# ielab/llm-rankers

Hardware: AMD Instinct MI355X
Metric: passages/sec (pointwise yes_no reranking, flan-t5-large shape) (higher is better)
Workload: dtype f16 (MFMA inputs), f32 accumulate + residual stream

## Files before the change

llm-rankers_amd/csrc/gemm.h:

```cpp
#pragma once
#include "common.h"
#include <type_traits>

enum GemmEpi { EPI_STORE_F16 = 0, EPI_RESID_F32 = 1, EPI_GEGLU_F16 = 2, EPI_RELU_F16 = 3, EPI_STORE_F32 = 4, EPI_SWIGLU_F16 = 5,
               EPI_ARGMAX_F32 = 6,
               EPI_LSE_F32 = 7 };
#define EPI_IS_GATED(E) ((E) == EPI_GEGLU_F16 || (E) == EPI_SWIGLU_F16)

struct GemmArgs {
  const half_t* A;
  const half_t* W;
  void* C;
  int lda, ldw, ldc;
  int M, N, K;
  int n_split;
  long split_stride;
  float scale;
  long bsA, bsW, bsC;
  const float* rowscale;
  half_t* xraw; float* ssq; int ldx, nb; float xs;
  const float* ssq_in; int nb_in; float eps_in;
  int* amax_idx;
  const int* lse_labels; int lse_npos; float* lse_xlab;
  int group_n;
// ... 371 lines not shown
      }
#pragma unroll
      for (int ni = 0; ni < 2; ++ni)
#pragma unroll
        for (int mi = 0; mi < 2; ++mi)
          acc[ni][mi] = __builtin_amdgcn_mfma_f32_32x32x16_f16(wf[ni], af[mi], acc[ni][mi], 0, 0, 0);
    }
    if (!GLDS && more) {
      gemm_write_tile(nA, wave, lane, ra);
      gemm_write_tile(nW, wave, lane, rw);
    }
  }

  if (EPI == EPI_RESID_F32) {
#pragma unroll
    for (int i = 0; i < 2; ++i)
#pragma unroll
      for (int j = 0; j < 2; ++j)
#pragma unroll
        for (int r = 0; r < 16; ++r) acc[i][j][r] = acc[i][j][r] * p.scale + res[i][j][r];
  }
  __syncthreads();
  if (EPI == EPI_RESID_F32) {
    GemmArgs q = p; q.scale = 1.f;
    float rsc[2] = {1.f, 1.f};
    gemm_epilogue_staged<EPI, 2, 2, true>(q, acc, m0 + wm * 64, n0 + wn * 64, lane, gemm_smem + wave * (32 * (64 * 4 + 16)), rsc);
  } else {
    float rsc[2];
    gemm_row_factors<2>(p, m0 + wm * 64, l31, rsc);
    gemm_epilogue_staged<EPI, 2, 2>(p, acc, m0 + wm * 64, n0 + wn * 64, lane, gemm_smem + wave * (32 * (64 * 4 + 16)), rsc);
  }
}

template <int EPI, int NST>
__global__ __launch_bounds__(128, NST == 4 ? 2 : (NST == 3 ? 3 : 4)) void gemm_s64_kernel(GemmArgs p) {
  extern __shared__ __attribute__((aligned(16))) unsigned char gemm_smem[];
  half_t* smem = (half_t*)gemm_smem;
  constexpr int TILE = 64 * 64;
  const int tid = threadIdx.x, lane = tid & 63;
  const int wave = __builtin_amdgcn_readfirstlane(tid >> 6);
  const int l31 = lane & 31, hh = lane >> 5;
  const int tiles_m = (p.M + 63) >> 6, tiles_n = (p.N + 63) >> 6;
  int tm, tn;
  gemm_tile_coords(blockIdx.x, tiles_m, tiles_n, tm, tn);
  const int m0 = tm * 64, n0 = tn * 64;
  const half_t* srcA[4];
  const half_t* srcW[4];
#pragma unroll
  for (int i = 0; i < 4; ++i) {
    const int pslot = (wave * 4 + i) * 64 + lane;
    const int r = pslot >> 3, c = pslot & 7;
    const int sw = (c ^ ((r >> 1) & 7)) << 3;
    const int ga = m0 + r < p.M ? m0 + r : p.M - 1, gw = n0 + r < p.N ? n0 + r : p.N - 1;
    srcA[i] = p.A + (size_t)ga * p.lda + sw;
    srcW[i] = p.W + (size_t)gw * p.ldw + sw;
  }
  auto stage = [&](int buf, int kt) {
    half_t* sA = smem + buf * 2 * TILE;
#pragma unroll
    for (int i = 0; i < 4; ++i)
      __builtin_amdgcn_global_load_lds((const __attribute__((address_space(1))) void*)(srcA[i] + kt * 64),
                                       (__attribute__((address_space(3))) void*)(sA + (wave * 4 + i) * 512), 16, 0, 0);
#pragma unroll
    for (int i = 0; i < 4; ++i)
      __builtin_amdgcn_global_load_lds((const __attribute__((address_space(1))) void*)(srcW[i] + kt * 64),
                                       (__attribute__((address_space(3))) void*)(sA + TILE + (wave * 4 + i) * 512), 16, 0, 0);
  };
  f32x16 acc[2][1];
#pragma unroll
  for (int i = 0; i < 2; ++i)
#pragma unroll
    for (int r = 0; r < 16; ++r) acc[i][0][r] = 0.f;
  const int nk = p.K >> 6;
#pragma unroll
  for (int s = 0; s < NST - 1; ++s)
    if (s < nk) stage(s, s);
  int cur = 0, nxt = NST - 1;
  for (int kt = 0; kt < nk; ++kt) {
    const int younger = nk - 1 - kt < NST - 2 ? nk - 1 - kt : NST - 2;
    if (younger >= 2) asm volatile("s_waitcnt vmcnt(16)" ::: "memory");
    else if (younger == 1) asm volatile("s_waitcnt vmcnt(8)" ::: "memory");
    else asm volatile("s_waitcnt vmcnt(0)" ::: "memory");
    __builtin_amdgcn_s_barrier();
    __builtin_amdgcn_sched_barrier(0);
    if (kt + NST - 1 < nk) stage(nxt, kt + NST - 1);
    const half_t* sA = smem + cur * 2 * TILE;
    const half_t* sW = sA + TILE;
#pragma unroll
    for (int ks = 0; ks < 4; ++ks) {
      const int cc = ks * 2 + hh;
      const half8 af = gemm_frag(sA, wave * 32 + l31, cc);
#pragma unroll
      for (int ni = 0; ni < 2; ++ni)
        acc[ni][0] = __builtin_amdgcn_mfma_f32_32x32x16_f16(gemm_frag(sW, ni * 32 + l31, cc), af, acc[ni][0], 0, 0, 0);
    }
    cur = cur + 1 == NST ? 0 : cur + 1;
    nxt = nxt + 1 == NST ? 0 : nxt + 1;
  }
  __syncthreads();
  float rsc[1];
  gemm_row_factors<1>(p, m0 + wave * 32, l31, rsc);
  gemm_epilogue_staged<EPI, 2, 1>(p, acc, m0 + wave * 32, n0, lane, gemm_smem + wave * (32 * (64 * 4 + 16)), rsc);
}

#define SKINNY_THREADS 512
template <int EPI, int NT>
__global__ __launch_bounds__(SKINNY_THREADS) void gemm_skinny_kernel(GemmArgs p) {
  __shared__ float red[4 * NT * 1024];
  const int tid = threadIdx.x, wave = tid >> 6, lane = tid & 63;
  const int l31 = lane & 31, hh = lane >> 5;
  const int n0 = blockIdx.x * 32 * NT;
  const int nsteps = p.K >> 4;
  const int mrow0 = blockIdx.z * 32;
  const int m = mrow0 + l31 < p.M ? mrow0 + l31 : p.M - 1;
  p.A += (size_t)blockIdx.y * p.bsA;
  p.W += (size_t)blockIdx.y * p.bsW;
  p.C = (char*)p.C + (size_t)blockIdx.y * p.bsC * ((EPI == EPI_RESID_F32 || EPI == EPI_STORE_F32 || EPI == EPI_ARGMAX_F32) ? 4 : 2);
  const half_t* arow = p.A + (size_t)m * p.lda + 8 * hh;
  const half_t* wrow[NT];
#pragma unroll
  for (int t = 0; t < NT; ++t) {
    int n = n0 + t * 32 + l31;
    n = n < p.N ? n : p.N - 1;
    wrow[t] = p.W + (size_t)n * p.ldw + 8 * hh;
  }
  f32x16 acc[NT][1];
#pragma unroll
  for (int t = 0; t < NT; ++t)
#pragma unroll
    for (int r = 0; r < 16; ++r) acc[t][0][r] = 0.f;
// ... 548 lines not shown
```

llm-rankers_amd/csrc/rk_engine.hip:

```cpp
#include <hip/hip_runtime.h>
#include <dlfcn.h>
#include <rccl/rccl.h>

#include <algorithm>
#include <cmath>
#include <cstdarg>
#include <cstdio>
#include <cstring>
#include <map>
#include <atomic>
#include <string>
#include <vector>

#include "../../include/rk_engine.h"
#include "attention.h"
#include "decoder_kernels.h"
#include "gemm.h"
#include "gemv_rows.h"
#include "llama_kernels.h"
#include "misc_kernels.h"

namespace {

thread_local std::string g_create_error;
// ... 43 lines not shown
  float* dhidden = nullptr; half_t *dxn = nullptr, *dqkv = nullptr, *dctx = nullptr, *dq = nullptr, *dffh = nullptr, *dlast = nullptr;
  half_t* dxraw[2] = {nullptr, nullptr}; float* dssq[2] = {nullptr, nullptr}; float* drowscale = nullptr;
  float* dssq_few[2] = {nullptr, nullptr};
  half_t *xqk = nullptr, *xctx = nullptr;
  float *xpart = nullptr, *xstat = nullptr; bool have_cross_kv = false;
  float* d_scores = nullptr; float* h_scores = nullptr;
  int* h_small = nullptr;
  std::vector<int> cache_dec, cache_out, cache_rows;
  std::vector<int> cache_g2; unsigned long dec_epoch = 0, g2_epoch = ~0ul;
  hipEvent_t ev_enc = nullptr, ev_dec = nullptr; bool dec_pending = false;
};

struct rk_engine {
  rk_model_desc d{};
  int dev = 0;
  std::string err;
  bool finalized = false;
  int inner = 0;
  std::map<std::string, HostTensor> host;
  std::vector<void*> allocs;
  half_t *emb = nullptr, *lm_head = nullptr, *cross_kv_w = nullptr;
  std::vector<EncLayerW> enc;
  std::vector<DecLayerW> dec;
  float *enc_final_ln = nullptr, *dec_final_ln = nullptr, *lut_enc = nullptr, *lut_dec = nullptr;
  float* logits = nullptr; size_t logits_cap = 0;
  const int* lse_labels = nullptr; int lse_npos = 0; float* lse_xlab = nullptr;
  float* amax_val = nullptr; int* amax_idx = nullptr; size_t amax_rows = 0;
  size_t scores_cap = 0;
  Slot slots[RK_SLOTS];
  struct Options {
    int glds = 1, skinny = 0x3F, overlap = 1, gemm_variant = 0, attn_short = 5, xattn_direct = 1, attn_heads_per_wg = 0, attn_ko = 0,
        gemm_persistent = 1, fold_norm = 1, s64_stages = 0, dec_fold_norm = 1, greedy_spec = 160, consumer_stats = 1, xattn_mfma = 1,
        dec_ffn_tiled = 1, gemm_split = 1, dec_fuse = 1, dec_fuse_rows = 0, dec_attn_seq = 1, attn_long = 1, attn_long_nw = 0,
        llama_attn_dma = 1, attn_long_xcd = 1, llama_attn_nw = 0, dec_graph = 1, gemm_sk = 1, dec_cross_mfma = 1, dec_gemv = 1, dec_gemv_rows = 4;
  } opt;
  float* attn_trace = nullptr;
  int n_cu = 256;
  struct SkWs { hipStream_t st = nullptr; float* slabs = nullptr; int* cnt = nullptr; };
  SkWs sk_ws[2 * RK_SLOTS];
  hipEvent_t t0 = nullptr, t1 = nullptr, t_tmp = nullptr;
  bool prof_on = false;
  std::vector<ProfRec> prof_recs; size_t prof_used = 0;
  double prof_flops[PC_COUNT] = {0}, prof_bytes[PC_COUNT] = {0}; int64_t prof_n[PC_COUNT] = {0};
  int family = 0; rk_llama_desc ld{};
  float rope_factor = 0.f, rope_low = 1.f, rope_high = 4.f; int rope_orig = 0;
  std::vector<LlamaLayerW> ll; float *l_final_ln = nullptr, *rope_cos = nullptr, *rope_sin = nullptr; int* d_pos = nullptr;
  struct GraphEntry { int seen = 0; bool failed = false; hipGraphExec_t exec = nullptr; };
  std::map<std::vector<int>, GraphEntry> graphs; int opt_epoch = 0;
  ncclComm_t comm = nullptr; int comm_rank = 0, comm_world = 1;
  float* d_gather[RK_SLOTS] = {nullptr}; float* h_gather[RK_SLOTS] = {nullptr}; size_t gather_cap = 0;
  hipEvent_t ev_gather[RK_SLOTS] = {nullptr}; bool gather_pending[RK_SLOTS] = {false}; int gather_n[RK_SLOTS] = {0};
  float *d_gsend = nullptr, *d_gall = nullptr, *h_gall = nullptr, *h_gstage = nullptr;
  hipEvent_t ev_gall = nullptr, ev_append = nullptr; bool gall_pending = false, append_foreign = false; int gall_n = 0;
};

namespace {

int fail(rk_engine* e, int code, const char* fmt, ...) {
  char buf[1024];
  va_list ap;
  va_start(ap, fmt);
  vsnprintf(buf, sizeof buf, fmt, ap);
  va_end(ap);
  if (e) e->err = buf; else g_create_error = buf;
  return code;
}

// ... 54 lines not shown
template <int EPI, int WM, int WN, int MI, int NI>
void launch_v2(hipStream_t st, const GemmArgs& a) {
  constexpr int BM = WM * MI * 32, BN = WN * NI * 32;
  constexpr int smem_stages = 2 * (BM + BN) * 64 * 2, smem_epi = WM * WN * 32 * (NI * 32 * 4 + 16);
  constexpr int smem = smem_stages > smem_epi ? smem_stages : smem_epi;
  static std::atomic<uint64_t> attr_done{0};
  ensure_dynamic_lds((const void*)gemm_v2_kernel<EPI, WM, WN, MI, NI>, smem, attr_done);
  const int tiles = ((a.M + BM - 1) / BM) * ((a.N + BN - 1) / BN);
  hipLaunchKernelGGL((gemm_v2_kernel<EPI, WM, WN, MI, NI>), dim3(tiles), dim3(WM * WN * 64), smem, st, a);
}

#define KSPLIT_MAX_SLABS 256

template <int EPI, int KO = 0, bool RS = false, bool SPLIT = false>
void launch_pp2(hipStream_t st, const GemmArgs& a, int max_wgs) {
  constexpr int smem = 2 * 4 * 128 * 64 * 2 + 32768;
  static std::atomic<uint64_t> attr_done{0};
  ensure_dynamic_lds((const void*)gemm_pp2_kernel<EPI, KO, RS, SPLIT>, smem, attr_done);
  const int tiles = ((a.M + 255) / 256) * ((a.N + 255) / 256) * (SPLIT ? a.ksplit : 1);
  const int grid = max_wgs > 0 && tiles > max_wgs ? max_wgs : tiles;
  hipLaunchKernelGGL((gemm_pp2_kernel<EPI, KO, RS, SPLIT>), dim3(grid), dim3(512), smem, st, a);
}

int choose_ksplit(const rk_engine* e, int epi, int M, int N, int K) {
  if (!e->opt.gemm_sk || !(epi == EPI_RESID_F32 || epi == EPI_STORE_F32) || K % 64) return 1;
  const long tiles = (long)((M + 255) / 256) * ((N + 255) / 256);
  const int wgs = e->n_cu & ~7, nk = K / 64;
  if (e->opt.gemm_sk == 2)
    return (nk >= 4 && tiles * 2 <= KSPLIT_MAX_SLABS) ? 2 : 1;
  if (epi != EPI_RESID_F32 || tiles < 1 || tiles * 2 > wgs || nk < 96) return 1;
  return 2;
}

int choose_variant(const rk_engine* e, int epi, int M, int N, int K, bool fold_producer, double* cost_out) {
  *cost_out = 0;
  if (e->opt.gemm_variant) return (e->opt.gemm_variant == 3 && (EPI_IS_GATED(epi) || fold_producer)) ? 2 : e->opt.gemm_variant;
  struct V { int id, bm, bn, slots; double round_us; };
  static const V vs[5] = {{5, 256, 256, 256, 25.5}, {2, 256, 256, 256, 29.8}, {3, 256, 192, 256, 24.7}, {4, 256, 128, 256, 19.0}, {1, 128, 128, 512, 17.3}};
  if ((long)((M + 127) / 128) * ((N + 127) / 128) <= 192 && K >= 64) { *cost_out = 15.0; return 6; }
  double best = 1e30; int bv = 1;
  for (const V& v : vs) {
    if (v.id == 3 && (EPI_IS_GATED(epi) || fold_producer)) continue;
    if (v.id == 5 && K < 128) continue;
    const long tiles = (long)((M + v.bm - 1) / v.bm) * ((N + v.bn - 1) / v.bn);
    double cost = (double)((tiles + v.slots - 1) / v.slots) * v.round_us;
    if (v.id == 5 && e->opt.gemm_sk == 1 && choose_ksplit(e, epi, M, N, K) > 1) cost = 0.0;
    if (cost < best - 1e-9) { best = cost; bv = v.id; }
  }
  *cost_out = best;
  return bv;
}

#define RK_XRAW_SCALE 0.0625f
struct GemmFold { const float* rowscale = nullptr; half_t* xraw = nullptr; float* ssq = nullptr; const float* ssq_in = nullptr; int nb_in = 0; };

enum GemmFamily { GEMM_NONE = -1, GEMM_TILED, GEMM_STREAM, GEMM_GEMV };
constexpr bool gemv_has(int E) { return E == EPI_STORE_F16 || E == EPI_RESID_F32 || E == EPI_GEGLU_F16 || E == EPI_RELU_F16 || E == EPI_STORE_F32; }
constexpr bool stream_has(int E) { return E != EPI_LSE_F32; }
constexpr bool tiled_has(int E) { return E != EPI_ARGMAX_F32; }
inline bool gemv_fits(int M, int K) { return M <= GEMV_MAX_ROWS && K % 8 == 0 && K <= 512 * GEMV_MAX_PIECES; }

struct Gemm {
  int cls, epi; const half_t* A; int lda; const half_t* W; int ldw; void* C; int ldc, M, N, K;
  int n_split = 0; long split_stride = 0;
  int batch = 1; long bsA = 0, bsW = 0, bsC = 0;
  GemmFamily family = GEMM_TILED;
  GemmFold fold;
  Gemm(int cls_, int epi_, const half_t* A_, int lda_, const half_t* W_, int ldw_, void* C_, int ldc_, int M_, int N_, int K_)
      : cls(cls_), epi(epi_), A(A_), lda(lda_), W(W_), ldw(ldw_), C(C_), ldc(ldc_), M(M_), N(N_), K(K_) {}
  Gemm& heads(int b, long sA, long sW, long sC) { batch = b; bsA = sA; bsW = sW; bsC = sC; return *this; }
  Gemm& split(int n, long stride) { n_split = n; split_stride = stride; return *this; }
  Gemm& on(GemmFamily f) { family = f; return *this; }
  Gemm& with(const GemmFold& f) { fold = f; return *this; }
};

struct GemmPlan {
  GemmFamily family = GEMM_NONE;
  int nb = 0;
  int m_pp2 = 0, ks_pp2 = 1, variant = 0, ksplit = 1, stages = 0;
  int wgs = 0;
  int ko = 0;
  const rk_engine::SkWs* ks_ws = nullptr;
  bool pp2() const { return family == GEMM_TILED && (m_pp2 > 0 || variant == 5); }
};

GemmPlan plan_gemm(const rk_engine* e, const Gemm& c, hipStream_t st) {
  GemmPlan p;
  const int epi = c.epi, M = c.M, N = c.N, K = c.K;
  if (c.family == GEMM_GEMV) {
    if (gemv_has(epi) && gemv_fits(M, K) && c.batch == 1 && c.n_split == 0) {
      p.family = GEMM_GEMV;
      p.nb = gemv_grid(N, e->n_cu);
    }
    return p;
  }
  if ((c.family == GEMM_STREAM || c.batch > 1) && c.n_split == 0 && (((e->opt.skinny >> epi) & 1) || c.batch > 1 || epi == EPI_ARGMAX_F32)) {
    if (stream_has(epi)) { p.family = GEMM_STREAM; p.nb = (N + 31) / 32; }
    return p;
  }
  if (!tiled_has(epi)) return p;
  p.family = GEMM_TILED;
  p.nb = (N + 63) / 64;
  p.wgs = e->opt.gemm_persistent == 1 ? (e->n_cu & ~7) : (e->opt.gemm_persistent & ~7);
  for (const auto& w : e->sk_ws) if (!p.ks_ws && w.st == st && w.slabs) p.ks_ws = &w;
  auto ksplit = [&](int rows) { return e->opt.gemm_persistent == 1 && p.ks_ws ? choose_ksplit(e, epi, rows, N, K) : 1; };
  const bool fold_producer = c.fold.xraw != nullptr;
  double whole = 0;
  p.variant = choose_variant(e, epi, M, N, K, fold_producer, &whole);
  if (e->opt.gemm_split && !e->opt.gemm_variant && K >= 128 && e->opt.gemm_persistent == 1 &&
      (epi == EPI_STORE_F16 || epi == EPI_RESID_F32 || EPI_IS_GATED(epi) || epi == EPI_RELU_F16)) {
    const int tiles_n = (N + 255) / 256, tiles_m = (M + 255) / 256;
    const long rounds = (long)tiles_m * tiles_n / p.wgs;
    const int panels = (int)(rounds * p.wgs / tiles_n);
    if (rounds >= 1 && (long)tiles_m * tiles_n % p.wgs != 0 && panels >= 1 && panels < tiles_m) {
      const long used = (long)panels * tiles_n;
      double rest = 0;
      const int v_rest = choose_variant(e, epi, M - panels * 256, N, K, fold_producer, &rest);
      if ((double)((used + p.wgs - 1) / p.wgs) * 25.5 + rest + 1.5 < whole - 1e-9) {
        p.m_pp2 = panels * 256; p.ks_pp2 = ksplit(p.m_pp2); p.variant = v_rest;
      }
    }
  }
#ifdef RK_MEASURE
  if (epi == EPI_STORE_F16 && p.variant > 80 && p.variant <= 96 && K >= 128) { p.ko = p.variant - 80; p.variant = 5; return p; }
#endif
  if (p.variant > 6) p.variant = 5;
  if (p.variant == 5 && K < 128) p.variant = 2;
  if (p.variant == 5) p.ksplit = ksplit(M - p.m_pp2);
  if (p.variant == 6) {
    const int tiles = ((M - p.m_pp2 + 63) / 64) * ((N + 63) / 64);
    p.stages = e->opt.s64_stages;
    if (p.stages < 2 || p.stages > 4) p.stages = tiles <= 2 * e->n_cu ? 4 : (tiles <= 3 * e->n_cu ? 3 : 2);
  }
  return p;
}

template <int EPI, int NST>
void launch_s64(hipStream_t st, const GemmArgs& a) {
  constexpr int smem = NST * 16384;
  static std::atomic<uint64_t> attr_done{0};
  ensure_dynamic_lds((const void*)gemm_s64_kernel<EPI, NST>, smem, attr_done);
  hipLaunchKernelGGL((gemm_s64_kernel<EPI, NST>), dim3(((a.M + 63) / 64) * ((a.N + 63) / 64)), dim3(128), smem, st, a);
}

template <int EPI>
void launch_pp2_plan(hipStream_t st, GemmArgs a, const GemmPlan& p, int ks) {
#ifdef RK_MEASURE
  if constexpr (EPI == EPI_STORE_F16) {
    switch (p.ko) {
      case 0: break;
      case 8: launch_pp2<EPI, 8>(st, a, p.wgs); return;
      case 16: launch_pp2<EPI, 16>(st, a, p.wgs); return;
      case 1: launch_pp2<EPI, 1>(st, a, p.wgs); return;
      case 2: launch_pp2<EPI, 2>(st, a, p.wgs); return;
      case 3: launch_pp2<EPI, 3>(st, a, p.wgs); return;
      case 4: launch_pp2<EPI, 4>(st, a, p.wgs); return;
      case 5: launch_pp2<EPI, 5>(st, a, p.wgs); return;
      default: launch_pp2<EPI, 6>(st, a, p.wgs); return;
    }
  }
#endif
  if constexpr (EPI == EPI_STORE_F16 || EPI_IS_GATED(EPI) || EPI == EPI_RELU_F16) {
    if (a.rowscale) { launch_pp2<EPI, 0, true>(st, a, p.wgs); return; }
  }
  if constexpr (EPI == EPI_RESID_F32 || EPI == EPI_STORE_F32) {
    if (ks > 1) { a.ksplit = ks; a.ks_slabs = p.ks_ws->slabs; a.ks_cnt = p.ks_ws->cnt; launch_pp2<EPI, 0, false, true>(st, a, p.wgs); return; }
  }
  launch_pp2<EPI>(st, a, p.wgs);
}

template <int EPI>
void launch_tiled(const rk_engine* e, hipStream_t st, GemmArgs a, const GemmPlan& p) {
  if (p.m_pp2 > 0) {
    GemmArgs head = a;
    head.M = p.m_pp2;
    launch_pp2_plan<EPI>(st, head, p, p.ks_pp2);
    const size_t r = (size_t)p.m_pp2;
    constexpr size_t celt = (EPI == EPI_RESID_F32 || EPI == EPI_STORE_F32) ? 4 : 2;
    a.A += r * a.lda;
    a.C = (char*)a.C + r * (size_t)a.ldc * celt;
    if (a.rowscale) a.rowscale += r;
    if (a.xraw) a.xraw += r * a.ldx;
    if (a.ssq) a.ssq += r * a.nb;
    if (a.ssq_in) a.ssq_in += r * a.nb_in;
    a.M -= p.m_pp2;
  }
  switch (p.variant) {
    case 6:
      if (p.stages == 4) launch_s64<EPI, 4>(st, a);
      else if (p.stages == 3) launch_s64<EPI, 3>(st, a);
      else launch_s64<EPI, 2>(st, a);
      return;
    case 5: launch_pp2_plan<EPI>(st, a, p, p.ksplit); return;
    case 2: launch_v2<EPI, 2, 4, 4, 2>(st, a); return;
    case 3: if constexpr (!EPI_IS_GATED(EPI)) { launch_v2<EPI, 4, 2, 2, 3>(st, a); return; } break;
    case 4: launch_v2<EPI, 4, 2, 2, 2>(st, a); return;
  }
  const int tiles = ((a.M + GEMM_BM - 1) / GEMM_BM) * ((a.N + GEMM_BN - 1) / GEMM_BN);
  if (e->opt.glds)
    hipLaunchKernelGGL((gemm_f16_kernel<EPI, true>), dim3(tiles), dim3(256), GEMM_LDS_BYTES, st, a);
  else
    hipLaunchKernelGGL((gemm_f16_kernel<EPI, false>), dim3(tiles), dim3(256), GEMM_LDS_BYTES, st, a);
}

template <int EPI, int MR>
void launch_gemv(const rk_engine* e, hipStream_t st, const GemmArgs& a) {
  const int smem = MR * a.K * 2 + (GEMV_MAX_ROWS + 4 * GEMV_MAX_ROWS) * 4;
  static std::atomic<uint64_t> attr_done{0};
  if (smem > 65536) ensure_dynamic_lds((const void*)gemv_rows_kernel<EPI, MR>, 160 * 1024, attr_done);
  hipLaunchKernelGGL((gemv_rows_kernel<EPI, MR>), dim3(gemv_grid(EPI_IS_GATED(EPI) ? a.N / 2 : a.N, e->n_cu)), dim3(256), smem, st, a);
}

template <int EPI>
void launch_stream(hipStream_t st, const GemmArgs& a, int batch) {
  constexpr int NT = EPI_IS_GATED(EPI) ? 2 : 1;
  hipLaunchKernelGGL((gemm_skinny_kernel<EPI, NT>), dim3((a.N + 32 * NT - 1) / (32 * NT), batch, (a.M + 31) / 32), dim3(SKINNY_THREADS), 0, st, a);
}

// ... 2 lines not shown
  if (epi == E) f(std::integral_constant<int, E>());
  else if constexpr (E < EPI_LSE_F32) with_epi<E + 1>(epi, f);
}

int gemm(rk_engine* e, hipStream_t st, const Gemm& c, int* nb = nullptr) {
  if (c.M <= 0) return RK_OK;
  const GemmPlan p = plan_gemm(e, c, st);
  if (p.family == GEMM_NONE)
    return fail(e, RK_ERR_STATE, "no kernel of family %d takes the GEMM M=%d N=%d K=%d (epilogue %d, batch %d)", (int)c.family, c.M, c.N, c.K, c.epi, c.batch);
  if (nb) *nb = p.nb;
  GemmArgs a{c.A, c.W, c.C, c.lda, c.ldw, c.ldc, c.M, c.N, c.K, c.n_split, c.split_stride, 1.f, c.bsA, c.bsW, c.bsC};
  a.rowscale = c.fold.rowscale; a.xraw = c.fold.xraw; a.ssq = c.fold.ssq; a.ldx = c.N; a.nb = p.nb; a.xs = RK_XRAW_SCALE;
  a.ssq_in = c.fold.ssq_in; a.nb_in = c.fold.nb_in; a.eps_in = e->d.eps;
  a.group_n = GEMM_GROUP_N;
  if (c.epi == EPI_ARGMAX_F32) a.amax_idx = e->amax_idx;
  if (c.epi == EPI_LSE_F32) { a.lse_labels = e->lse_labels; a.lse_npos = e->lse_npos; a.lse_xlab = e->lse_xlab; }
  const double flops = 2.0 * c.M * (double)c.N * c.K * c.batch;
  const double out_elems = EPI_IS_GATED(c.epi) ? (double)c.M * c.N / 2 : (double)c.M * c.N;
  const double bytes = 2.0 * ((double)c.M * c.K + (double)c.N * c.K) +
                       out_elems * (c.epi == EPI_RESID_F32 ? 8.0 : (c.epi == EPI_STORE_F32 ? 4.0 : 2.0));
  Bracket br(e, st, c.cls, flops, bytes);
  with_epi(c.epi, [&](auto E) {
    constexpr int EPI = decltype(E)::value;
    if constexpr (gemv_has(EPI)) {
      if (p.family == GEMM_GEMV) {
        if (a.M <= 2) launch_gemv<EPI, 2>(e, st, a);
        else if (a.M <= 4) launch_gemv<EPI, 4>(e, st, a);
        else if (a.M <= 8) launch_gemv<EPI, 8>(e, st, a);
        else launch_gemv<EPI, 16>(e, st, a);
        return;
      }
    }
    if constexpr (stream_has(EPI)) { if (p.family == GEMM_STREAM) { launch_stream<EPI>(st, a, c.batch); return; } }
    if constexpr (tiled_has(EPI)) { if (p.family == GEMM_TILED) launch_tiled<EPI>(e, st, a, p); }
  });
  return RK_OK;
}

void rmsnorm(rk_engine* e, hipStream_t st, const float* x, const float* w, half_t* out, const int* row_map, int rows, float scale = 1.f) {
  if (rows <= 0) return;
  Bracket br(e, st, PC_NORM, 3.0 * rows * e->d.d_model, (double)rows * e->d.d_model * 6.0);
  const int dm = e->d.d_model;
  const dim3 g((rows + 3) / 4), b(256);
  if (dm <= 1024) hipLaunchKernelGGL(rmsnorm_kernel<4>, g, b, 0, st, x, w, out, row_map, rows, dm, e->d.eps, scale);
  else if (dm <= 2048) hipLaunchKernelGGL(rmsnorm_kernel<8>, g, b, 0, st, x, w, out, row_map, rows, dm, e->d.eps, scale);
  else hipLaunchKernelGGL(rmsnorm_kernel<16>, g, b, 0, st, x, w, out, row_map, rows, dm, e->d.eps, scale);
}

void embed(rk_engine* e, hipStream_t st, const int* ids, float* out, int rows, half_t* xraw = nullptr, float* rowscale = nullptr) {
  if (rows <= 0) return;
  Bracket br(e, st, PC_EMBED, 0, (double)rows * e->d.d_model * 6.0);
  hipLaunchKernelGGL(embed_gather_kernel, dim3((rows + 3) / 4), dim3(256), 0, st, ids, e->emb, out, rows,
                     e->d.d_model, e->d.vocab, xraw, rowscale, RK_XRAW_SCALE, e->d.eps);
}

void rowscale(rk_engine* e, hipStream_t st, const float* ssq, float* out, int rows, int nb) {
  if (rows <= 0) return;
  Bracket br(e, st, PC_NORM, 0, (double)rows * (nb + 1) * 4.0);
  hipLaunchKernelGGL(rowscale_kernel, dim3((rows + 255) / 256), dim3(256), 0, st, ssq, out, rows, nb, e->d.d_model, e->d.eps, RK_XRAW_SCALE);
}

int rel_bucket(int rel, bool bidirectional, int num_buckets, int max_distance) {
  int ret = 0;
  if (bidirectional) {
    num_buckets /= 2;
    if (rel > 0) ret += num_buckets;
// ... 107 lines not shown
        else if (nw == 6) { ensure_dynamic_lds((const void*)attn_enc_long_kernel<6>, ATTL_LDS_BYTES, attr6); hipLaunchKernelGGL(attn_enc_long_kernel<6>, grid, dim3(384), ATTL_LDS_BYTES, st, a); }
        else if (nw == 4) { ensure_dynamic_lds((const void*)attn_enc_long_kernel<4>, ATTL_LDS_BYTES, attr4); hipLaunchKernelGGL(attn_enc_long_kernel<4>, grid, dim3(256), ATTL_LDS_BYTES, st, a); }
        else { ensure_dynamic_lds((const void*)attn_enc_long_kernel<3>, ATTL_LDS_BYTES, attr3); hipLaunchKernelGGL(attn_enc_long_kernel<3>, grid, dim3(192), ATTL_LDS_BYTES, st, a); }
      }
      else
        hipLaunchKernelGGL(attn_enc_kernel, dim3((sl.maxL + 127) / 128, d.n_heads, sl.n_seq), dim3(256), 0, st, a);
    }
    RC(gemm(e, st, Gemm(PC_ENC_GEMM_O, EPI_RESID_F32, sl.ctx, I, w.o, I, sl.hidden, dm, T, dm, I).with(prod), &nb));
    RC(gemm(e, st, normed(w.ln1, Gemm(PC_ENC_GEMM_FFN_IN, d.gated_gelu ? EPI_GEGLU_F16 : EPI_RELU_F16, xin, dm, fold ? w.ffn_in_f : w.ffn_in, dm,
                                      sl.ffh, F, T, d.gated_gelu ? 2 * F : F, dm))));
    RC(gemm(e, st, Gemm(PC_ENC_GEMM_FFN_OUT, EPI_RESID_F32, sl.ffh, F, w.ffn_out, F, sl.hidden, dm, T, dm, F).with(last ? GemmFold() : prod), &nb));
  }
  rmsnorm(e, st, sl.hidden, e->enc_final_ln, sl.enc_out, nullptr, T);
  if (need_cross_kv)
    RC(gemm(e, st, Gemm(PC_GEMM_CROSS_KV, EPI_STORE_F16, sl.enc_out, dm, e->cross_kv_w, dm, sl.cross_kv, 2 * I, T, d.n_dec_layers * 2 * I, dm)
                       .split(2 * I, (long)d.max_tokens * 2 * I)));
  sl.have_cross_kv = need_cross_kv;
  HIPCHK(e, hipGetLastError());
  return RK_OK;
}

struct DecTree { int rows; const int* keys; const int* pos; const int* seq; };
int run_decoder(rk_engine* e, Slot& sl, int Ld, const DecTree* tree = nullptr) {
  const rk_model_desc& d = e->d;
  hipStream_t st = dec_stream(e, sl);
  const int B = sl.n_seq, M = tree ? tree->rows : B * Ld, I = e->inner, dm = d.d_model, F = d.d_ff;
  if (tree && (sl.have_cross_kv || Ld < 2)) return fail(e, RK_ERR_STATE, "the tree form needs the query-side cross-attention and L_d >= 2");
  const bool ws = Ld <= 4;
  const bool dfold = ws && e->opt.dec_fold_norm && (e->opt.skinny & 0x3F) == 0x3F;
  const bool fuse_any = (e->opt.dec_fuse == 2 || (e->opt.dec_fuse == 1 && Ld == 1));
  const bool few = dfold && e->opt.dec_gemv && Ld >= 2 && M <= e->opt.dec_gemv_rows && !fuse_any &&
                   gemv_fits(M, dm) && gemv_fits(M, I) && gemv_fits(M, F);
  const GemmFamily fam = few ? GEMM_GEMV : (ws ? GEMM_STREAM : GEMM_TILED);
  float* const* ssq = few ? sl.dssq_few : sl.dssq;
  int cur = 0, nb = 0, rc = RK_OK;
  auto xin = [&]() { return dfold ? sl.dxraw[cur] : sl.dxn; };
  auto norm = [&](const float* ln) {
    GemmFold f;
    if (!dfold) rmsnorm(e, st, sl.dhidden, ln, sl.dxn, nullptr, M);
    else if (!nb) f.rowscale = sl.drowscale;
    else { f.ssq_in = ssq[cur]; f.nb_in = nb; }
    return f;
  };
  auto resid = [&](Gemm c, bool stats = true) {
    if (!(dfold && stats)) return gemm(e, st, c.on(fam));
    c.fold.xraw = sl.dxraw[cur ^ 1]; c.fold.ssq = ssq[cur ^ 1];
    cur ^= 1;
    return gemm(e, st, c.on(fam), &nb);
  };
  embed(e, st, sl.d_dec_ids, sl.dhidden, M, dfold ? sl.dxraw[0] : nullptr, dfold ? sl.drowscale : nullptr);
  const size_t smem_self = (64 + 256 + 8 + (size_t)Ld) * sizeof(float);
  const size_t smem_cross = (64 + 256 + 8 + (size_t)sl.maxL) * sizeof(float);
  for (int l = 0; l < d.n_dec_layers; ++l) {
    const DecLayerW& w = e->dec[l];
    const GemmFold in0 = norm(w.ln0);
    if (Ld == 1) {
      RC(resid(Gemm(PC_DEC_GEMM, EPI_RESID_F32, xin(), dm, dfold ? w.ov_f : w.ov, dm, sl.dhidden, dm, M, dm, dm).with(in0)));
    } else {
      RC(gemm(e, st, Gemm(PC_DEC_GEMM, EPI_STORE_F16, xin(), dm, dfold ? w.qkv_f : w.qkv, dm, sl.dqkv, 3 * I, M, 3 * I, dm).on(fam).with(in0)));
      AttnDecArgs a{sl.dqkv, 3 * I, sl.dqkv + I, sl.dqkv + 2 * I, 3 * I, nullptr, sl.dctx, I, e->lut_dec, Ld, 1, Ld};
      {
        Bracket br(e, st, PC_DEC_ATTN, 4.0 * M * Ld * I, 0);
        if (tree) {
          a.tree_keys = tree->keys; a.tree_pos = tree->pos;
          hipLaunchKernelGGL(attn_dec_kernel, dim3(1, d.n_heads, M), dim3(256), smem_self, st, a);
        } else if (e->opt.dec_cross_mfma && Ld > XA_MAX_LD && Ld <= ATTX_MAXQ) {
          hipLaunchKernelGGL(attn_dec_cross_mfma_kernel, dim3(d.n_heads, B), dim3(128), ATTX_LDS_BYTES, st, a);
        } else if (e->opt.dec_attn_seq && attn_dec_seq_lds(Ld) <= 160 * 1024) {
          hipLaunchKernelGGL(attn_dec_seq_kernel, dim3(d.n_heads, B), dim3(256), attn_dec_seq_lds(Ld), st, a);
        } else {
          hipLaunchKernelGGL(attn_dec_kernel, dim3(Ld, d.n_heads, B), dim3(256), smem_self, st, a);
        }
      }
      RC(resid(Gemm(PC_DEC_GEMM, EPI_RESID_F32, sl.dctx, I, w.o, I, sl.dhidden, dm, M, dm, I)));
    }
    const bool fuse = (e->opt.dec_fuse == 2 || (e->opt.dec_fuse == 1 && Ld == 1)) && !sl.have_cross_kv && dm % 128 == 0;
    const GemmFold in1 = norm(w.ln1);
    if (!fuse) RC(gemm(e, st, Gemm(PC_DEC_GEMM, EPI_STORE_F16, xin(), dm, dfold ? w.cq_f : w.cq, dm, sl.dq, I, M, I, dm).on(fam).with(in1)));
    if (!sl.have_cross_kv) {
      const int H = d.n_heads, nch = (sl.maxL + 63) / 64;
      const int blk = std::max(1, std::min(XA_MAX_ROWS, XA_MAX_CHUNKS / nch));
// ... 1311 lines not shown

}

namespace {
struct OptionDesc { const char* key; int rk_engine::Options::*field; int lo, hi; const char* allowed; const char* what; };
const OptionDesc kOptions[] = {
  {"dec_graph", &rk_engine::Options::dec_graph, 0, 1, nullptr, "decoder chains replayed as HIP graphs (1) or launched eagerly (0)"},
  {"gemm_glds", &rk_engine::Options::glds, 0, 1, nullptr, "128x128 GEMM staging by LDS-DMA (1) or through registers (0); same bits"},
  {"gemm_skinny", &rk_engine::Options::skinny, 0, 0x3F, nullptr, "bit per epilogue kind: few-row GEMMs on the weight-streaming kernel (1 = all)"},
  {"dec_ffn_tiled", &rk_engine::Options::dec_ffn_tiled, 0, 1, nullptr, "one-position decoder: FFN-in on the tiled kernels (1) or the weight-streaming kernel (0)"},
  {"gemm_persistent", &rk_engine::Options::gemm_persistent, 0, 1024, nullptr, "ping-pong GEMM: 1 = one workgroup per CU walks the tiles, 0 = one per tile, n > 1 = n workgroups"},
  {"gemm_s64_stages", &rk_engine::Options::s64_stages, 0, 4, "0,2,3,4", "LDS stages of the 64x64 GEMM (0 = from the tile count); same bits"},
  {"consumer_stats", &rk_engine::Options::consumer_stats, 0, 1, nullptr, "encoder row factors formed by the non-persistent consumer GEMMs themselves (1) or always by rowscale_kernel (0); same bits"},
  {"greedy_spec", &rk_engine::Options::greedy_spec, 0, 65536, nullptr, "rk_t5_greedy2: most decoder rows of a speculative pass; 0 = never speculate; same tokens"},
  {"dec_fold_norm", &rk_engine::Options::dec_fold_norm, 0, 1, nullptr, "decoder RMSNorms folded into the weight-streaming GEMMs (1) or separate kernels (0)"},
  {"fold_norm", &rk_engine::Options::fold_norm, 0, 1, nullptr, "encoder RMSNorm folded into the GEMMs (1) or separate kernels (0)"},
  {"xattn_mfma", &rk_engine::Options::xattn_mfma, 0, 1, nullptr, "query-side cross-attention: weighted sums on the matrix cores (1) or the VALU form (0)"},
  {"attn_heads_per_wg", &rk_engine::Options::attn_heads_per_wg, 0, 4096, nullptr, "short-sequence attention: (sequence, head) items per wave group, 0 = dealt evenly; same bits"},
  {"xattn_direct", &rk_engine::Options::xattn_direct, 0, 1, nullptr, "decoder prefixes <= 16: query-side cross-attention (1) or materialised K / V (0)"},
  {"attn_short", &rk_engine::Options::attn_short, 0, 6, "0,5,6", "sequences <= 192 keys: DMA kernel with two (5) / one (6) wave group per workgroup, or the tiled kernel (0); same bits"},
  {"gemm_variant", &rk_engine::Options::gemm_variant, 0, 120, nullptr, "tile variant: 0 auto, 1..6 see choose_variant; measurement builds: 80+ / 100+ knock-outs"},
  {"dec_fuse_rows", &rk_engine::Options::dec_fuse_rows, 0, 32, nullptr, "rows per workgroup of dec_cross_qk_kernel (0 = auto); same bits"},
  {"dec_fuse", &rk_engine::Options::dec_fuse, 0, 2, nullptr, "few-row decoder: projections around the query-side cross-attention fused at one position (1), always (2), never (0)"},
  {"llama_attn_nw", &rk_engine::Options::llama_attn_nw, 0, 8, "0,4,8", "waves per workgroup of the Llama LDS-DMA attention kernel (0 = default 8); same bits"},
  {"llama_attn_dma", &rk_engine::Options::llama_attn_dma, 0, 1, nullptr, "Llama causal attention: LDS-DMA kernel (1) or the register-staged first kernel (0); differ within fp16 noise"},
  {"attn_long_xcd", &rk_engine::Options::attn_long_xcd, 0, 1, nullptr, "long-sequence attention: workgroups of a (sequence, head) pair on one XCD (1) or dealt over all eight (0); same bits"},
  {"attn_long_nw", &rk_engine::Options::attn_long_nw, 0, 12, "0,3,4,6,12", "waves per workgroup of the long-sequence attention kernel (0 = default 4); same bits"},
  {"attn_long", &rk_engine::Options::attn_long, 0, 1, nullptr, "sequences > 192 keys: the chunked LDS-DMA kernel (1) or the tiled kernel (0)"},
  {"dec_gemv", &rk_engine::Options::dec_gemv, 0, 1, nullptr, "decoder pass of at most 16 rows at >= 2 positions (one setwise compare): plain projections on the wave-per-column GEMV kernel (1) or the weight-streaming MFMA kernel (0); differ within fp32 summation-order noise"},
  {"dec_gemv_rows", &rk_engine::Options::dec_gemv_rows, 1, GEMV_MAX_ROWS, nullptr, "largest row count of a decoder pass that takes the few-row GEMV family (default 4 = the measured cross-over; the kernel takes up to 16)"},
  {"dec_cross_mfma", &rk_engine::Options::dec_cross_mfma, 0, 1, nullptr, "long decoder prefixes (qlm), cross-attention over the materialised K / V: matrix-core kernel for sequences <= 192 keys (1) or the staged fma-chain kernels (0); differ within fp16 noise"},
  {"dec_attn_seq", &rk_engine::Options::dec_attn_seq, 0, 1, nullptr, "decoder attention at several positions: one workgroup per (head, sequence) (1) or per query row (0); same bits"},
  {"gemm_sk", &rk_engine::Options::gemm_sk, 0, 2, nullptr, "ping-pong GEMM, fp32 residual projections with few tiles and a long K: K split over two workgroups (1: choose_ksplit), never (0), wherever it fits (2: tests)"},
  {"gemm_split", &rk_engine::Options::gemm_split, 0, 1, nullptr, "rows beyond the ping-pong kernel's last whole round on a fill-in tile variant (1) or one launch (0); same bits"},
#ifdef RK_MEASURE
  {"attn_ko", &rk_engine::Options::attn_ko, 0, 1 << 20, nullptr, "timing-only knock-outs of the attention kernels (measurement builds)"},
#endif
};
bool option_value_ok(const OptionDesc& o, int value) {
  if (value < o.lo || value > o.hi) return false;
  if (!o.allowed) return true;
  for (const char* p = o.allowed; *p;) {
    if (atoi(p) == value) return true;
    while (*p && *p != ',') ++p;
    if (*p == ',') ++p;
  }
  return false;
}
}

extern "C" {

int rk_engine_set_option(rk_engine* e, const char* key, int value) {
  if (!e || !key) return RK_ERR_INVALID;
  if (!strcmp(key, "overlap")) {
    if (value < 0 || value > 1) return fail(e, RK_ERR_INVALID, "option overlap: 0..1");
    if (set_device(e) || sync_all(e)) return RK_ERR_HIP;
    for (Slot& sl : e->slots) sl.dec_pending = false;
    e->opt.overlap = value;
    e->opt_epoch++;
    return RK_OK;
  }
#ifdef RK_MEASURE
  if (!strcmp(key, "attn_trace")) {
    if (value && !e->attn_trace) { if (hipMalloc(&e->attn_trace, 12 * 16 * 16 * sizeof(float)) != hipSuccess) return RK_ERR_HIP; hipMemset(e->attn_trace, 0, 12 * 16 * 16 * sizeof(float)); }
    if (!value && e->attn_trace) { hipFree(e->attn_trace); e->attn_trace = nullptr; }
// ... 124 lines not shown
```

Before: 7321.

## Route one-position decoder residual projections through K-split 64x64 tile GEMM

Adds a split-K mode to the 64x64 tile kernel. Each split writes fp32 partials to global slabs, and the last-arriving workgroup per tile (found with an atomic counter) sums them and runs the residual epilogue. The pointwise one-position folded decoder now sends its residual projections to this path instead of the weight-streaming kernel. The aim is more workgroups and better CU use for small-M projections with long K, at the cost of extra slab traffic, an atomic handshake, and a different summation order.

```diff
diff --git a/llm-rankers_amd/csrc/gemm.h b/llm-rankers_amd/csrc/gemm.h
--- a/llm-rankers_amd/csrc/gemm.h
+++ b/llm-rankers_amd/csrc/gemm.h
@@ -427,7 +427,8 @@
   }
 }
 
-template <int EPI, int NST>
+#define S64_KSPLIT_MAX 8
+template <int EPI, int NST, int KS = 1>
 __global__ __launch_bounds__(128, NST == 4 ? 2 : (NST == 3 ? 3 : 4)) void gemm_s64_kernel(GemmArgs p) {
   extern __shared__ __attribute__((aligned(16))) unsigned char gemm_smem[];
   half_t* smem = (half_t*)gemm_smem;
@@ -436,8 +437,16 @@
   const int wave = __builtin_amdgcn_readfirstlane(tid >> 6);
   const int l31 = lane & 31, hh = lane >> 5;
   const int tiles_m = (p.M + 63) >> 6, tiles_n = (p.N + 63) >> 6;
+  int tile = blockIdx.x, sp = 0, kt0 = 0, nk = p.K >> 6;
+  if constexpr (KS > 1) {
+    const int ntiles = tiles_m * tiles_n, base = nk / KS, rem = nk - base * KS;
+    sp = tile / ntiles;
+    tile -= sp * ntiles;
+    kt0 = sp * base + (sp < rem ? sp : rem);
+    nk = base + (sp < rem ? 1 : 0);
+  }
   int tm, tn;
-  gemm_tile_coords(blockIdx.x, tiles_m, tiles_n, tm, tn);
+  gemm_tile_coords(tile, tiles_m, tiles_n, tm, tn);
   const int m0 = tm * 64, n0 = tn * 64;
   const half_t* srcA[4];
   const half_t* srcW[4];
@@ -447,8 +456,8 @@
     const int r = pslot >> 3, c = pslot & 7;
     const int sw = (c ^ ((r >> 1) & 7)) << 3;
     const int ga = m0 + r < p.M ? m0 + r : p.M - 1, gw = n0 + r < p.N ? n0 + r : p.N - 1;
-    srcA[i] = p.A + (size_t)ga * p.lda + sw;
-    srcW[i] = p.W + (size_t)gw * p.ldw + sw;
+    srcA[i] = p.A + (size_t)ga * p.lda + kt0 * 64 + sw;
+    srcW[i] = p.W + (size_t)gw * p.ldw + kt0 * 64 + sw;
   }
   auto stage = [&](int buf, int kt) {
     half_t* sA = smem + buf * 2 * TILE;
@@ -466,7 +475,6 @@
   for (int i = 0; i < 2; ++i)
 #pragma unroll
     for (int r = 0; r < 16; ++r) acc[i][0][r] = 0.f;
-  const int nk = p.K >> 6;
 #pragma unroll
   for (int s = 0; s < NST - 1; ++s)
     if (s < nk) stage(s, s);
@@ -491,6 +499,56 @@
     }
     cur = cur + 1 == NST ? 0 : cur + 1;
     nxt = nxt + 1 == NST ? 0 : nxt + 1;
+  }
+  if constexpr (KS > 1) {
+    __shared__ int flag;
+    const int ntiles = tiles_m * tiles_n;
+    const unsigned lane_off = (unsigned)(wave * 8 * 64 + lane) * 4;
+    {
+      float* mine = p.ks_slabs + (size_t)(sp * ntiles + tile) * 4096 + lane_off;
+#pragma unroll
+      for (int f = 0; f < 8; ++f) {
+        const f32x16& a = acc[f >> 2][0];
+        const int q = f & 3;
+        const f32x4 x = {a[4 * q], a[4 * q + 1], a[4 * q + 2], a[4 * q + 3]};
+        asm volatile("s_nop 4\n\tglobal_store_dwordx4 %0, %1, off sc1\n\ts_nop 1" :: "v"(mine + f * 256), "v"(x) : "memory");
+      }
+      asm volatile("s_waitcnt vmcnt(0)" ::: "memory");
+    }
+    __syncthreads();
+    if (tid == 0) {
+      const int last = __hip_atomic_fetch_add(p.ks_cnt + tile, 1, __ATOMIC_RELAXED, __HIP_MEMORY_SCOPE_AGENT) == KS - 1;
+      if (last) {
+        __hip_atomic_store(p.ks_cnt + tile, 0, __ATOMIC_RELAXED, __HIP_MEMORY_SCOPE_AGENT);
+        __builtin_amdgcn_fence(__ATOMIC_ACQUIRE, "agent");
+      }
+      flag = last;
+    }
+    __syncthreads();
+    if (!flag) return;
+    constexpr int GP = KS >= 8 ? 2 : 4;
+#pragma unroll
+    for (int g = 0; g < 8 / GP; ++g) {
+      f32x4 x[KS][GP];
+#pragma unroll
+      for (int s = 0; s < KS; ++s)
+#pragma unroll
+        for (int i = 0; i < GP; ++i) {
+          const float* slab = p.ks_slabs + (size_t)(s * ntiles + tile) * 4096;
+          x[s][i] = *(const f32x4*)(slab + lane_off + (g * GP + i) * 256);
+        }
+#pragma unroll
+      for (int i = 0; i < GP; ++i) {
+        const int f = g * GP + i;
+        f32x4 t = x[0][i];
+#pragma unroll
+        for (int s = 1; s < KS; ++s) t = f32x4{t[0] + x[s][i][0], t[1] + x[s][i][1], t[2] + x[s][i][2], t[3] + x[s][i][3]};
+        asm volatile("" : "+v"(t));
+#pragma unroll
+        for (int j = 0; j < 4; ++j) acc[f >> 2][0][4 * (f & 3) + j] = t[j];
+      }
+      __builtin_amdgcn_sched_barrier(0);
+    }
   }
   __syncthreads();
   float rsc[1];
diff --git a/llm-rankers_amd/csrc/rk_engine.hip b/llm-rankers_amd/csrc/rk_engine.hip
--- a/llm-rankers_amd/csrc/rk_engine.hip
+++ b/llm-rankers_amd/csrc/rk_engine.hip
@@ -99,7 +99,8 @@
     int glds = 1, skinny = 0x3F, overlap = 1, gemm_variant = 0, attn_short = 5, xattn_direct = 1, attn_heads_per_wg = 0, attn_ko = 0,
         gemm_persistent = 1, fold_norm = 1, s64_stages = 0, dec_fold_norm = 1, greedy_spec = 160, consumer_stats = 1, xattn_mfma = 1,
         dec_ffn_tiled = 1, gemm_split = 1, dec_fuse = 1, dec_fuse_rows = 0, dec_attn_seq = 1, attn_long = 1, attn_long_nw = 0,
-        llama_attn_dma = 1, attn_long_xcd = 1, llama_attn_nw = 0, dec_graph = 1, gemm_sk = 1, dec_cross_mfma = 1, dec_gemv = 1, dec_gemv_rows = 4;
+        llama_attn_dma = 1, attn_long_xcd = 1, llama_attn_nw = 0, dec_graph = 1, gemm_sk = 1, dec_cross_mfma = 1, dec_gemv = 1, dec_gemv_rows = 4,
+        dec_onepos = 1, dec_onepos_ks = 0;
   } opt;
   float* attn_trace = nullptr;
   int n_cu = 256;
@@ -220,6 +221,11 @@
   return 2;
 }
 
+int choose_ksplit64(const rk_engine* e, int K) {
+  if (e->opt.dec_onepos_ks > 0) return e->opt.dec_onepos_ks;
+  return K / 64 >= 8 ? 2 : 1;
+}
+
 int choose_variant(const rk_engine* e, int epi, int M, int N, int K, bool fold_producer, double* cost_out) {
   *cost_out = 0;
   if (e->opt.gemm_variant) return (e->opt.gemm_variant == 3 && (EPI_IS_GATED(epi) || fold_producer)) ? 2 : e->opt.gemm_variant;
@@ -242,7 +248,7 @@
 #define RK_XRAW_SCALE 0.0625f
 struct GemmFold { const float* rowscale = nullptr; half_t* xraw = nullptr; float* ssq = nullptr; const float* ssq_in = nullptr; int nb_in = 0; };
 
-enum GemmFamily { GEMM_NONE = -1, GEMM_TILED, GEMM_STREAM, GEMM_GEMV };
+enum GemmFamily { GEMM_NONE = -1, GEMM_TILED, GEMM_STREAM, GEMM_GEMV, GEMM_KSPLIT };
 constexpr bool gemv_has(int E) { return E == EPI_STORE_F16 || E == EPI_RESID_F32 || E == EPI_GEGLU_F16 || E == EPI_RELU_F16 || E == EPI_STORE_F32; }
 constexpr bool stream_has(int E) { return E != EPI_LSE_F32; }
 constexpr bool tiled_has(int E) { return E != EPI_ARGMAX_F32; }
@@ -279,6 +285,15 @@
     if (gemv_has(epi) && gemv_fits(M, K) && c.batch == 1 && c.n_split == 0) {
       p.family = GEMM_GEMV;
       p.nb = gemv_grid(N, e->n_cu);
+    }
+    return p;
+  }
+  if (c.family == GEMM_KSPLIT) {
+    for (const auto& w : e->sk_ws) if (!p.ks_ws && w.st == st && w.slabs) p.ks_ws = &w;
+    p.ksplit = choose_ksplit64(e, K);
+    if (epi == EPI_RESID_F32 && c.batch == 1 && c.n_split == 0 && K % 64 == 0 && K / 64 >= p.ksplit && p.ks_ws && (N + 63) / 64 <= KSPLIT_MAX_SLABS) {
+      p.family = GEMM_KSPLIT;
+      p.nb = (N + 63) / 64;
     }
     return p;
   }
@@ -323,12 +338,39 @@
   return p;
 }
 
-template <int EPI, int NST>
+template <int EPI, int NST, int KS = 1>
 void launch_s64(hipStream_t st, const GemmArgs& a) {
   constexpr int smem = NST * 16384;
   static std::atomic<uint64_t> attr_done{0};
-  ensure_dynamic_lds((const void*)gemm_s64_kernel<EPI, NST>, smem, attr_done);
-  hipLaunchKernelGGL((gemm_s64_kernel<EPI, NST>), dim3(((a.M + 63) / 64) * ((a.N + 63) / 64)), dim3(128), smem, st, a);
+  ensure_dynamic_lds((const void*)gemm_s64_kernel<EPI, NST, KS>, smem, attr_done);
+  hipLaunchKernelGGL((gemm_s64_kernel<EPI, NST, KS>), dim3(((a.M + 63) / 64) * ((a.N + 63) / 64) * KS), dim3(128), smem, st, a);
+}
+
+template <int EPI>
+GemmArgs from_row(GemmArgs a, int r) {
+  constexpr size_t celt = (EPI == EPI_RESID_F32 || EPI == EPI_STORE_F32) ? 4 : 2;
+  a.A += (size_t)r * a.lda;
+  a.C = (char*)a.C + (size_t)r * a.ldc * celt;
+  if (a.rowscale) a.rowscale += r;
+  if (a.xraw) a.xraw += (size_t)r * a.ldx;
+  if (a.ssq) a.ssq += (size_t)r * a.nb;
+  if (a.ssq_in) a.ssq_in += (size_t)r * a.nb_in;
+  a.M -= r;
+  return a;
+}
+
+void launch_ksplit(hipStream_t st, GemmArgs a, const GemmPlan& p) {
+  const int tiles_n = (a.N + 63) / 64;
+  const int panels = std::min(KSPLIT_MAX_SLABS / tiles_n, KSPLIT_MAX_SLABS * 16 / (tiles_n * p.ksplit));
+  a.ksplit = p.ksplit; a.ks_slabs = p.ks_ws->slabs; a.ks_cnt = p.ks_ws->cnt;
+  for (int r = 0; r < a.M; r += 64 * panels) {
+    GemmArgs b = from_row<EPI_RESID_F32>(a, r);
+    b.M = std::min(b.M, 64 * panels);
+    if (p.ksplit == 8) launch_s64<EPI_RESID_F32, 4, 8>(st, b);
+    else if (p.ksplit == 4) launch_s64<EPI_RESID_F32, 4, 4>(st, b);
+    else if (p.ksplit == 2) launch_s64<EPI_RESID_F32, 4, 2>(st, b);
+    else launch_s64<EPI_RESID_F32, 4>(st, b);
+  }
 }
 
 template <int EPI>
@@ -363,15 +405,7 @@
     GemmArgs head = a;
     head.M = p.m_pp2;
     launch_pp2_plan<EPI>(st, head, p, p.ks_pp2);
-    const size_t r = (size_t)p.m_pp2;
-    constexpr size_t celt = (EPI == EPI_RESID_F32 || EPI == EPI_STORE_F32) ? 4 : 2;
-    a.A += r * a.lda;
-    a.C = (char*)a.C + r * (size_t)a.ldc * celt;
-    if (a.rowscale) a.rowscale += r;
-    if (a.xraw) a.xraw += r * a.ldx;
-    if (a.ssq) a.ssq += r * a.nb;
-    if (a.ssq_in) a.ssq_in += r * a.nb_in;
-    a.M -= p.m_pp2;
+    a = from_row<EPI>(a, p.m_pp2);
   }
   switch (p.variant) {
     case 6:
@@ -440,6 +474,7 @@
       }
     }
     if constexpr (stream_has(EPI)) { if (p.family == GEMM_STREAM) { launch_stream<EPI>(st, a, c.batch); return; } }
+    if constexpr (EPI == EPI_RESID_F32) { if (p.family == GEMM_KSPLIT) { launch_ksplit(st, a, p); return; } }
     if constexpr (tiled_has(EPI)) { if (p.family == GEMM_TILED) launch_tiled<EPI>(e, st, a, p); }
   });
   return RK_OK;
@@ -613,6 +648,8 @@
   const bool few = dfold && e->opt.dec_gemv && Ld >= 2 && M <= e->opt.dec_gemv_rows && !fuse_any &&
                    gemv_fits(M, dm) && gemv_fits(M, I) && gemv_fits(M, F);
   const GemmFamily fam = few ? GEMM_GEMV : (ws ? GEMM_STREAM : GEMM_TILED);
+  const bool onepos = e->opt.dec_onepos && Ld == 1 && !tree && dfold && !sl.have_cross_kv && fuse_any && dm % 128 == 0;
+  const GemmFamily fam_res = onepos ? GEMM_KSPLIT : fam;
   float* const* ssq = few ? sl.dssq_few : sl.dssq;
   int cur = 0, nb = 0, rc = RK_OK;
   auto xin = [&]() { return dfold ? sl.dxraw[cur] : sl.dxn; };
@@ -624,10 +661,10 @@
     return f;
   };
   auto resid = [&](Gemm c, bool stats = true) {
-    if (!(dfold && stats)) return gemm(e, st, c.on(fam));
+    if (!(dfold && stats)) return gemm(e, st, c.on(fam_res));
     c.fold.xraw = sl.dxraw[cur ^ 1]; c.fold.ssq = ssq[cur ^ 1];
     cur ^= 1;
-    return gemm(e, st, c.on(fam), &nb);
+    return gemm(e, st, c.on(fam_res), &nb);
   };
   embed(e, st, sl.d_dec_ids, sl.dhidden, M, dfold ? sl.dxraw[0] : nullptr, dfold ? sl.drowscale : nullptr);
   const size_t smem_self = (64 + 256 + 8 + (size_t)Ld) * sizeof(float);
@@ -2005,6 +2042,8 @@
   {"dec_cross_mfma", &rk_engine::Options::dec_cross_mfma, 0, 1, nullptr, "long decoder prefixes (qlm), cross-attention over the materialised K / V: matrix-core kernel for sequences <= 192 keys (1) or the staged fma-chain kernels (0); differ within fp16 noise"},
   {"dec_attn_seq", &rk_engine::Options::dec_attn_seq, 0, 1, nullptr, "decoder attention at several positions: one workgroup per (head, sequence) (1) or per query row (0); same bits"},
   {"gemm_sk", &rk_engine::Options::gemm_sk, 0, 2, nullptr, "ping-pong GEMM, fp32 residual projections with few tiles and a long K: K split over two workgroups (1: choose_ksplit), never (0), wherever it fits (2: tests)"},
+  {"dec_onepos", &rk_engine::Options::dec_onepos, 0, 1, nullptr, "one-position folded decoder (pointwise): the three residual projections per layer on 64x64 tiles with a K split fixed by (N, K) (1) or the weight-streaming kernel (0); differ within fp32 summation-order noise"},
+  {"dec_onepos_ks", &rk_engine::Options::dec_onepos_ks, 0, S64_KSPLIT_MAX, "0,1,2,4,8", "measurement: K split of dec_onepos's projections (0 = choose_ksplit64; forcing it changes the last bits)"},
   {"gemm_split", &rk_engine::Options::gemm_split, 0, 1, nullptr, "rows beyond the ping-pong kernel's last whole round on a fill-in tile variant (1) or one launch (0); same bits"},
 #ifdef RK_MEASURE
   {"attn_ko", &rk_engine::Options::attn_ko, 0, 1 << 20, nullptr, "timing-only knock-outs of the attention kernels (measurement builds)"},
```

Result: no change. 7316 (median of 3 runs) (-0.1%).
